# numz/ComfyUI-SeedVR2_VideoUpscaler

Hardware: NVIDIA H100
Metric: upscaled frames/sec SeedVR2-3B 720p->4K (higher is better)
Workload: dtype bf16

## Files before the change

comfyui-seedvr2_videoupscaler_b200/csrc/gemm.cu:

```cuda
#include <cuda.h>
#include <cuda_runtime.h>
#include <cuda_bf16.h>
#include <stdint.h>
#include <stdio.h>
#include <stdlib.h>

#include <type_traits>

#include "ptx.cuh"
#include "svr2_internal.h"

namespace svr2 {

constexpr int BLOCK_M = 128;
constexpr int BLOCK_K = 64;
constexpr int WGMMA_K = 16;

struct GemmParams {
  int M, N, K;
  int num_m_tiles, num_n_tiles, num_k_blocks;
  int band_h;
  int group_n;
  int a_mode;
  int tiles_w, tiles_h;
// ... 34 lines not shown
  const float* qk_weight;
  float qk_eps;
  int qkv_inner;
};

enum : int {
  EPI_BIAS = 1,
  EPI_GATE = 2,
  EPI_RESIDUAL = 4,
  EPI_SWIGLU = 8,
  EPI_GELU = 16,
  EPI_F32 = 32,
  EPI_SHUFFLE = 64,
  EPI_SILU = 128,
  EPI_ROWSTAT = 256,
  EPI_PEXP = 512,
  EPI_ROWSCALE = 1024,
};

template <int BLOCK_N, bool EPI_WG>
struct SmemLayout {
  static constexpr int kABytes = BLOCK_M * BLOCK_K * 2;
  static constexpr int kBBytes = BLOCK_N * BLOCK_K * 2;
  static constexpr int kStageBytes = kABytes + kBBytes;
  static constexpr int kTileCols = BLOCK_N < 32 ? 32 : BLOCK_N;
  static constexpr int kStagingBytes = EPI_WG ? BLOCK_M * kTileCols * 2 : 8 * 4096;
  static constexpr int kBudget = 232448 - kStagingBytes - 256 - 1024;
  static constexpr int kStages = kBudget / kStageBytes > 8 ? 8 : kBudget / kStageBytes;
  static constexpr int kStagingOffset = kStages * kStageBytes;
  static constexpr int kBarOffset = kStagingOffset + kStagingBytes;
  static constexpr int kTotal = kBarOffset + 256 + 1024;
};

__device__ __forceinline__ void acc_ld32(const float* acc, uint32_t idx, uint32_t (&v)[32]) {
  const float4* s = reinterpret_cast<const float4*>(acc + idx);
#pragma unroll
  for (int i = 0; i < 8; ++i) {
    const float4 t = s[i];
    v[4 * i] = __float_as_uint(t.x); v[4 * i + 1] = __float_as_uint(t.y);
    v[4 * i + 2] = __float_as_uint(t.z); v[4 * i + 3] = __float_as_uint(t.w);
  }
}

__device__ __forceinline__ void stat_acc(float4& a, const uint4& d) {
  const uint32_t w[4] = {d.x, d.y, d.z, d.w};
#pragma unroll
  for (int e = 0; e < 4; ++e) {
    const float lo = __uint_as_float(w[e] << 16), hi = __uint_as_float(w[e] & 0xffff0000u);
    if (e < 2) { a.x += lo + hi; a.y += lo * lo + hi * hi; }
    else { a.z += lo + hi; a.w += lo * lo + hi * hi; }
  }
}

__device__ __forceinline__ uint4 add_bf16x8(const uint4& a, const uint4& b) {
  const uint32_t aw[4] = {a.x, a.y, a.z, a.w}, bw[4] = {b.x, b.y, b.z, b.w};
  uint32_t o[4];
#pragma unroll
  for (int e = 0; e < 4; ++e)
    o[e] = pack_bf16x2(__uint_as_float(aw[e] << 16) + __uint_as_float(bw[e] << 16),
                       __uint_as_float(aw[e] & 0xffff0000u) + __uint_as_float(bw[e] & 0xffff0000u));
  return make_uint4(o[0], o[1], o[2], o[3]);
}

__device__ __forceinline__ void conv_tile(const GemmParams& p, int m_blk, int& t_o, int& th, int& tw) {
  const int full = p.T_out * p.band_h * p.tiles_w;
  const int band = m_blk / full;
// ... 50 lines not shown
    const int m = m_blk * BLOCK_M + row;
    d.valid = m < p.M;
    const int hw = p.shuf_H * p.shuf_W;
    const int f = m / hw, rr = m - f * hw, h = rr / p.shuf_W, w = rr - h * p.shuf_W;
    const int grp = (n_blk * BLOCK_N) / p.shuf_c;
    const int z = grp % p.shuf_z, y = (grp / p.shuf_z) & 1, x = grp / (p.shuf_z * 2);
    int t_out = f * p.shuf_z + z;
    if (p.shuf_drop) {
      if (f == 0 && z == 1) d.valid = 0;
      if (f > 0) t_out -= 1;
    }
    const int Wo = p.shuf_W * 2;
    const long long pix = (long long)(2 * h + x) * Wo + (2 * w + y);
    d.off = (long long)(t_out + p.out_t_pad) * p.out_frame_stride + pix * p.ldc + ((n_blk * BLOCK_N) % p.shuf_c);
    d.dup = (p.out_dup_head && t_out == 0 && d.valid) ? 1 : 0;
  } else if (p.a_mode == 0) {
    const int m = m_blk * BLOCK_M + row;
    d.valid = m < p.M;
    d.off = (long long)m * p.ldc + (long long)n_blk * n_cols;
  } else {
    int t_o, th, tw;
    conv_tile(p, m_blk, t_o, th, tw);
    const int rh = row / p.bw;
    const int h = th * p.bh + rh;
    const int w = tw * p.bw + (row - rh * p.bw);
    d.valid = (h < p.H_out) && (w < p.W_out);
    d.off = (long long)(t_o + p.out_t_pad) * p.out_frame_stride + ((long long)h * p.W_out + w) * p.ldc +
            (long long)n_blk * BLOCK_N;
    d.dup = (p.out_dup_head && t_o == 0 && d.valid) ? 1 : 0;
  }
  return d;
}

template <int BLOCK_N, int KIND, bool SWAP = false, int EPI_CT = -1>
__global__ void __launch_bounds__(kNumThreads, 1)
gemm_wgmma_kernel(const __grid_constant__ CUtensorMap tmap_a, const __grid_constant__ CUtensorMap tmap_b,
                  const __grid_constant__ CUtensorMap tmap_a2, const GemmParams p) {
  if (p.run_if != nullptr && *p.run_if == 0) return;
  constexpr bool EPI_WG = kEpiWG<KIND>;
  static_assert(EPI_WG || (!SWAP && EPI_CT < 0), "swap-AB and compile-time epilogues are KIND_BF16 only");
  using L = SmemLayout<BLOCK_N, EPI_WG>;
  constexpr int kStages = L::kStages;
  constexpr int ACC_STRIDE = BLOCK_N < 32 ? 32 : BLOCK_N;
  constexpr int ACC_LD = ACC_STRIDE + 4;
  static_assert(EPI_WG || BLOCK_M * ACC_LD * 4 <= L::kStagingOffset, "the accumulator tile overlays the operand ring");
  extern __shared__ uint8_t smem_raw[];
  uint8_t* smem = reinterpret_cast<uint8_t*>((reinterpret_cast<uintptr_t>(smem_raw) + 1023) & ~uintptr_t(1023));
  uint64_t* full_bar = reinterpret_cast<uint64_t*>(smem + L::kBarOffset);
  uint64_t* empty_bar = full_bar + kStages;
  uint64_t* acc_free = empty_bar + kStages;
  uint64_t* tile_full = acc_free + 1;
  uint64_t* tile_empty = acc_free + 2;
  const float* acc_s = reinterpret_cast<const float*>(smem);
  uint8_t* tile_s = smem + L::kStagingOffset;

  const int warp = threadIdx.x >> 5;
  const int lane = threadIdx.x & 31;

  if (warp == 0 && lane == 0) {
    tma_prefetch_desc(&tmap_a);
    tma_prefetch_desc(&tmap_b);
    if (p.extra_blocks) tma_prefetch_desc(&tmap_a2);
  }
  if (warp == 1 && lane == 0) {
    for (int i = 0; i < kStages; ++i) {
      mbar_init(&full_bar[i], 1);
      mbar_init(&empty_bar[i], 2);
    }
    if constexpr (EPI_WG) {
      mbar_init(tile_full, 256);
      mbar_init(tile_empty, 32 * kEpiWarps);
    } else {
      mbar_init(acc_free, 256);
    }
    fence_barrier_init();
  }
  __syncthreads();

  const int num_n_tiles = p.num_n_tiles;
  const int num_m_tiles = p.num_m_tiles;
  const int num_tiles = num_m_tiles * num_n_tiles;
  const int tile0 = (int)blockIdx.x;
  const int tile_step = (int)gridDim.x;

  if (warp == 0 || warp == 3) {
    if (lane == 0) {
      int stage = 0;
      uint32_t phase = 0;
      uint32_t g = (warp == 0) ? 0u : 1u;
      uint32_t it = 0;
      const int a_mode = p.a_mode;
      const int nkb = p.num_k_blocks;
      auto acquire = [&](uint8_t*& sa, uint64_t*& fb) -> bool {
        const bool mine = (g++ & 1u) == 0u;
        if (mine) {
          mbar_wait(&empty_bar[stage], phase ^ 1);
          sa = smem + stage * L::kStageBytes;
          fb = &full_bar[stage];
          mbar_expect_tx(fb, L::kStageBytes);
        }
        return mine;
      };
      auto advance = [&]() {
        if (++stage == kStages) { stage = 0; phase ^= 1; }
      };
      auto tile_start = [&]() {
        if (!EPI_WG && it > 0) mbar_wait(acc_free, (it - 1) & 1u);
        ++it;
      };
      if (a_mode == 0) {
        for (int tile = tile0; tile < num_tiles; tile += tile_step) {
          int m_blk, n_blk;
          tile_coords(tile, num_m_tiles, num_n_tiles, p.group_n, m_blk, n_blk);
          tile_start();
          const int m0 = m_blk * BLOCK_M, n0 = n_blk * BLOCK_N;
          for (int kb = 0; kb < nkb; ++kb) {
            uint8_t* sa; uint64_t* fb;
            if (acquire(sa, fb)) {
              tma_load_2d(sa, &tmap_a, fb, kb * BLOCK_K, m0);
// ... 59 lines not shown
  } else if (warp >= 4) {
    const int wg = (warp - 4) >> 2;
    int mstage = 0;
    uint32_t mphase = 0;
    uint32_t it = 0;
    auto mainloop = [&](int nkb, auto&& tail) {
      float d[BLOCK_N / 2];
#pragma unroll
      for (int i = 0; i < BLOCK_N / 2; ++i) d[i] = 0.f;
      const bool leader = (threadIdx.x & 127) == 0;
      int prev = -1;
      for (int kb = 0; kb < nkb; ++kb) {
        mbar_wait(&full_bar[mstage], mphase);
        const uint32_t a_addr = smem_u32(smem + mstage * L::kStageBytes);
        const uint64_t a_desc = wgmma_desc_kmajor_sw128(a_addr + wg * 64 * 128);
        const uint64_t b_desc = wgmma_desc_kmajor_sw128(a_addr + L::kABytes);
        wgmma_fence_regs(d);
        wgmma_fence();
#pragma unroll
        for (int k = 0; k < BLOCK_K / WGMMA_K; ++k)
          wgmma_ss<BLOCK_N>(d, a_desc + uint64_t(k * 2), b_desc + uint64_t(k * 2), (kb | k) != 0);
        wgmma_commit();
        wgmma_fence_regs(d);
        wgmma_wait<1>();
        if (prev >= 0 && leader) mbar_arrive(&empty_bar[prev]);
        prev = mstage;
        if (++mstage == kStages) { mstage = 0; mphase ^= 1; }
      }
      wgmma_wait<0>();
      wgmma_fence_regs(d);
      if (prev >= 0 && leader) mbar_arrive(&empty_bar[prev]);
      tail(d);
    };
    const int epi = EPI_CT >= 0 ? EPI_CT : p.epi;
    const __nv_bfloat16* __restrict__ bias = p.bias;
    if constexpr (EPI_WG) {
      const int r0 = wg * 64 + ((warp & 3) << 4);
      const uint32_t tbase = smem_u32(tile_s);
      const int lr = lane & 7, mj = lane >> 3;
      auto store_tile = [&](float (&d)[BLOCK_N / 2], int n_blk) {
        if (it > 0) mbar_wait(tile_empty, (it - 1) & 1u);
        if constexpr (SWAP) {
          const int co = n_blk * BLOCK_M + r0 + (lane >> 2);
          const bool has_bias = (epi & EPI_BIAS) != 0;
          const float b0 = (has_bias && co < p.N) ? __bfloat162float(bias[co]) : 0.f;
          const float b1 = (has_bias && co + 8 < p.N) ? __bfloat162float(bias[co + 8]) : 0.f;
          const int chunk = (r0 >> 3) + (mj & 1);
#pragma unroll
          for (int i = 0; i < BLOCK_N / 2; i += 8) {
            const int pix = (i >> 3) * 16 + ((mj >> 1) << 3) + lr;
            stmatrix_x4_trans(tbase + pix * 256 + ((chunk ^ swap_tile_swz(pix)) << 4),
                              pack_bf16x2(d[i] + b0, d[i + 1] + b0), pack_bf16x2(d[i + 2] + b1, d[i + 3] + b1),
                              pack_bf16x2(d[i + 4] + b0, d[i + 5] + b0), pack_bf16x2(d[i + 6] + b1, d[i + 7] + b1));
          }
        } else {
          constexpr int ROW_B = L::kTileCols * 2;
          constexpr int SWZ = (L::kTileCols / 8 < 8 ? L::kTileCols / 8 : 8) - 1;
          const int row = r0 + ((mj & 1) << 3) + lr;
          const int cn0 = n_blk * BLOCK_N + 2 * (lane & 3);
#pragma unroll
          for (int i = 0; i < BLOCK_N / 2; i += 8) {
            float x[8];
#pragma unroll
            for (int e = 0; e < 8; ++e) x[e] = d[i + e];
            if (epi & EPI_BIAS) {
              const int cn = cn0 + (i >> 3) * 16;
              const uint32_t bl = cn < p.N ? __ldg(reinterpret_cast<const unsigned int*>(bias + cn)) : 0u;
              const uint32_t bh = cn + 8 < p.N ? __ldg(reinterpret_cast<const unsigned int*>(bias + cn + 8)) : 0u;
              x[0] += __uint_as_float(bl << 16); x[1] += __uint_as_float(bl & 0xffff0000u);
              x[2] += __uint_as_float(bl << 16); x[3] += __uint_as_float(bl & 0xffff0000u);
              x[4] += __uint_as_float(bh << 16); x[5] += __uint_as_float(bh & 0xffff0000u);
              x[6] += __uint_as_float(bh << 16); x[7] += __uint_as_float(bh & 0xffff0000u);
            }
            const int chunk = (i >> 3) * 2 + (mj >> 1);
            stmatrix_x4(tbase + row * ROW_B + ((chunk ^ (row & SWZ)) << 4), pack_bf16x2(x[0], x[1]),
                        pack_bf16x2(x[2], x[3]), pack_bf16x2(x[4], x[5]), pack_bf16x2(x[6], x[7]));
          }
        }
        mbar_arrive(tile_full);
      };
      for (int tile = tile0; tile < num_tiles; tile += tile_step, ++it) {
        int m_blk, n_blk;
        tile_coords(tile, num_m_tiles, num_n_tiles, p.group_n, m_blk, n_blk);
        mainloop(conv_k_blocks(p, m_blk), [&](float (&d)[BLOCK_N / 2]) { store_tile(d, n_blk); });
      }
    } else {
      auto acc_to_smem = [&](float (&d)[BLOCK_N / 2]) {
        named_bar_sync(1, 256);
        float* acc_w = reinterpret_cast<float*>(smem);
        const int r0 = wg * 64 + ((warp & 3) << 4) + (lane >> 2);
#pragma unroll
        for (int i = 0; i < BLOCK_N / 2; i += 4) {
          const int col = (i >> 2) * 8 + 2 * (lane & 3);
          *reinterpret_cast<float2*>(acc_w + r0 * ACC_LD + col) = make_float2(d[i], d[i + 1]);
          *reinterpret_cast<float2*>(acc_w + (r0 + 8) * ACC_LD + col) = make_float2(d[i + 2], d[i + 3]);
        }
        named_bar_sync(1, 256);
      };
      constexpr bool IS_BF16 = KIND == KIND_BF16_RS;
      constexpr bool IS_PEXP = KIND == KIND_PEXP || KIND == KIND_PEXP_STAT;
      constexpr int N_COLS = KIND == KIND_SWIGLU ? ACC_STRIDE / 2 : ACC_STRIDE;
      constexpr int COLS_W = N_COLS >= 64 ? N_COLS / 2 : N_COLS;
      constexpr int PH_COLS = KIND == KIND_F32 ? 32 : (COLS_W < 64 ? COLS_W : 64);
      constexpr int CPR = KIND == KIND_F32 ? PH_COLS / 4 : PH_COLS / 8;
      constexpr int ROWS_PER_IT = 32 / CPR;
      constexpr int N_IT = 32 / ROWS_PER_IT;
      constexpr int kBatch = N_IT < 4 ? N_IT : 4;
      const int q = warp & 3;
      const int half = (warp - 4) >> 2;
      const int row = q * 32 + lane;
      const bool active = (N_COLS >= 64) || (half == 0);
      const int col_lo = (N_COLS >= 64) ? half * COLS_W : 0;
      uint8_t* slab = smem + L::kStagingOffset + (warp - 4) * 4096;
      const int n_lim = KIND == KIND_SWIGLU ? p.N / 2 : p.N;
      const float* __restrict__ gate = p.gate;
      const __nv_bfloat16* __restrict__ resid = p.residual;
      for (int tile = tile0; tile < num_tiles; tile += tile_step) {
// ... 511 lines not shown
  cuuint32_t bdim[5], estr[5];
  for (int i = 0; i < rank; ++i) {
    gdim[i] = dims[i];
    bdim[i] = box[i];
    estr[i] = 1;
    if (i > 0) gstr[i - 1] = strides_bytes[i - 1];
  }
  CUresult r = enc(map, CU_TENSOR_MAP_DATA_TYPE_BFLOAT16, rank, const_cast<void*>(base), gdim, gstr, bdim, estr,
                   CU_TENSOR_MAP_INTERLEAVE_NONE, CU_TENSOR_MAP_SWIZZLE_128B, CU_TENSOR_MAP_L2_PROMOTION_L2_256B,
                   CU_TENSOR_MAP_FLOAT_OOB_FILL_NONE);
  if (r != CUDA_SUCCESS) {
    char msg[256];
    snprintf(msg, sizeof msg, "cuTensorMapEncodeTiled failed (%d) rank=%d dims=%llu,%llu,%llu box=%u,%u,%u", (int)r,
             rank, (unsigned long long)dims[0], (unsigned long long)(rank > 1 ? dims[1] : 0),
             (unsigned long long)(rank > 2 ? dims[2] : 0), box[0], rank > 1 ? box[1] : 0, rank > 2 ? box[2] : 0);
    return set_error(SVR2_ERR_CUDA, msg);
  }
  return SVR2_OK;
}

constexpr int kMaxDevices = 64;
int current_device() {
  int dev = 0;
  cudaGetDevice(&dev);
  return (dev >= 0 && dev < kMaxDevices) ? dev : 0;
}
static int g_num_sms[kMaxDevices] = {};
int num_sms() {
  const int dev = current_device();
  if (!g_num_sms[dev]) cudaDeviceGetAttribute(&g_num_sms[dev], cudaDevAttrMultiProcessorCount, dev);
  return g_num_sms[dev];
}

template <int BLOCK_N, int KIND, bool SWAP = false, int EPI_CT = -1>
static int launch_gemm(const CUtensorMap& ta, const CUtensorMap& tb, const GemmParams& p_in, cudaStream_t stream,
                       const CUtensorMap* ta2_opt = nullptr) {
  const CUtensorMap& ta2 = ta2_opt ? *ta2_opt : ta;
  using L = SmemLayout<BLOCK_N, kEpiWG<KIND>>;
  auto kern = gemm_wgmma_kernel<BLOCK_N, KIND, SWAP, EPI_CT>;
  GemmParams p = p_in;
  {
    const long long b_tile_bytes = (long long)(SWAP ? BLOCK_M : BLOCK_N) * p.num_k_blocks * BLOCK_K * 2;
    long long g = (16LL << 20) / (b_tile_bytes > 0 ? b_tile_bytes : 1);
    if (g < 1) g = 1;
    if (g > p.num_n_tiles) g = p.num_n_tiles;
    p.group_n = (int)g;
  }
  static bool configured[kMaxDevices] = {};
  const int dev = current_device();
  if (!configured[dev]) {
    cudaError_t e = cudaFuncSetAttribute(kern, cudaFuncAttributeMaxDynamicSharedMemorySize, L::kTotal);
    if (e != cudaSuccess) return set_error(SVR2_ERR_CUDA, cudaGetErrorString(e));
    configured[dev] = true;
  }
  int tiles = p.num_m_tiles * p.num_n_tiles;
  int grid = tiles < num_sms() ? tiles : num_sms();
  if (grid <= 0) return SVR2_OK;
  kern<<<grid, kNumThreads, L::kTotal, stream>>>(ta, tb, ta2, p);
  cudaError_t e = cudaGetLastError();
  if (e != cudaSuccess) return set_error(SVR2_ERR_CUDA, cudaGetErrorString(e));
  return SVR2_OK;
}

static int dispatch_gemm(int block_n, const CUtensorMap& ta, const CUtensorMap& tb, const GemmParams& p,
                         cudaStream_t s, const CUtensorMap* ta2 = nullptr) {
  if (ta2) {
    switch (block_n) {
      case 256: return launch_gemm<256, KIND_BF16>(ta, tb, p, s, ta2);
      case 128: return launch_gemm<128, KIND_BF16>(ta, tb, p, s, ta2);
    }
    return set_error(SVR2_ERR_ARG, "fused shortcut: Cout must be >= 128");
  }
// ... 192 lines not shown
extern "C" int svr2_conv3d_stats_bf16(const void* x, int T_in_total, int H, int W, int Cin, const void* w, int Cout,
                                      int kt, int kh, int kw, int stride_t, int stride_hw, int pad_hw, int T_out,
                                      int epi_flags, const void* bias, const void* residual, void* y, int out_t_pad,
                                      int out_dup_head, int ldc, void* stat_partial, int64_t stat_bytes,
                                      int* stat_slots, void* stream) {
  if (!stat_slots) return set_error(SVR2_ERR_ARG, "svr2_conv3d_stats_bf16: stat_slots must not be NULL");
  return conv3d_impl(x, T_in_total, H, W, Cin, w, Cout, kt, kh, kw, stride_t, stride_hw, pad_hw, T_out, epi_flags, bias,
                     residual, y, out_t_pad, out_dup_head, ldc, stat_partial, stat_bytes, stat_slots, stream);
}

extern "C" int svr2_conv3d_shortcut_stats_bf16(const void* x, int T_in_total, int H, int W, int Cin, const void* w,
                                               int Cout, int kt, int kh, int kw, int T_out, const void* bias,
                                               const void* x2, int C2, void* y, int out_t_pad, int out_dup_head,
                                               void* stat_partial, int64_t stat_bytes, int* stat_slots, void* stream) {
  if (!x2 || C2 <= 0 || (C2 % 64)) return set_error(SVR2_ERR_ARG, "svr2_conv3d_shortcut_stats_bf16: x2 / C2 % 64");
  if (Cout < 128) return set_error(SVR2_ERR_ARG, "svr2_conv3d_shortcut_stats_bf16: Cout must be >= 128");
  return conv3d_impl(x, T_in_total, H, W, Cin, w, Cout, kt, kh, kw, 1, 1, 1, T_out, EPI_BIAS, bias, nullptr, y,
                     out_t_pad, out_dup_head, Cout, stat_partial, stat_bytes, stat_slots, stream, x2, C2);
}

static void conv_tile_shape(int Cout, int H_out, int W_out, bool* swap_out, int* bw_out, int* bh_out) {
  const bool swap = (Cout > 64 && Cout <= 128) && (long long)H_out * W_out >= 256;
  int bw = 16, bh = 8;
  if (swap) {
    bw = 32; bh = 8;
    if (W_out <= 16) { bw = 16; bh = 16; }
    if (W_out <= 8) { bw = 8; bh = 32; }
  } else {
    if (W_out >= 128 && H_out < 8) { bw = 128; bh = 1; }
    else if (W_out <= 8) { bw = 8; bh = 16; }
  }
  *swap_out = swap; *bw_out = bw; *bh_out = bh;
}
extern "C" int svr2_conv_stat_slots(int Cout, int H_out, int W_out) {
  bool swap;
  int bw, bh;
  conv_tile_shape(Cout, H_out, W_out, &swap, &bw, &bh);
  return ((W_out + bw - 1) / bw) * ((H_out + bh - 1) / bh) * (swap ? 2 : 4);
}

static int conv3d_impl(const void* x, int T_in_total, int H, int W, int Cin, const void* w, int Cout, int kt,
                       int kh, int kw, int stride_t, int stride_hw, int pad_hw, int T_out, int epi_flags,
                       const void* bias, const void* residual, void* y, int out_t_pad, int out_dup_head,
                       int ldc, void* stat_partial, int64_t stat_bytes, int* stat_slots_out, void* stream,
                       const void* x2, int C2) {
  if (Cin % 64) return set_error(SVR2_ERR_ARG, "svr2_conv3d_bf16: Cin must be a multiple of 64 (pad channels)");
  if (Cout % 8 || ldc % 8) return set_error(SVR2_ERR_ARG, "svr2_conv3d_bf16: Cout/ldc must be multiples of 8");
  if (stride_hw != 1 && stride_hw != 2) return set_error(SVR2_ERR_ARG, "stride_hw must be 1 or 2");
  const int H_out = stride_hw == 1 ? H : H / 2, W_out = stride_hw == 1 ? W : W / 2;
  if (stride_hw == 2 && ((H | W) & 1)) return set_error(SVR2_ERR_ARG, "stride-2 conv needs even H, W");
  bool swap;
  int bw, bh;
  conv_tile_shape(Cout, H_out, W_out, &swap, &bw, &bh);
  const int bn = swap ? 128 : pick_block_n(Cout, 0);
  CUtensorMap ta, tb;
  int rc;
  if (stride_hw == 1) {
    uint64_t d[4] = {(uint64_t)Cin, (uint64_t)W, (uint64_t)H, (uint64_t)T_in_total};
    uint64_t s[3] = {(uint64_t)Cin * 2, (uint64_t)W * Cin * 2, (uint64_t)H * W * Cin * 2};
    uint32_t b[4] = {BLOCK_K, (uint32_t)bw, (uint32_t)bh, 1};
    rc = make_tmap_bf16(&ta, x, 4, d, s, b);
  } else {
    uint64_t d[5] = {(uint64_t)Cin * 2, (uint64_t)W / 2, 2, (uint64_t)H / 2, (uint64_t)T_in_total};
    uint64_t s[4] = {(uint64_t)Cin * 4, (uint64_t)W * Cin * 2, (uint64_t)W * Cin * 4, (uint64_t)H * W * Cin * 2};
    uint32_t b[5] = {BLOCK_K, (uint32_t)bw, 1, (uint32_t)bh, 1};
    rc = make_tmap_bf16(&ta, x, 5, d, s, b);
  }
  if (rc) return rc;
  CUtensorMap ta2;
  if (x2) {
    uint64_t d[4] = {(uint64_t)C2, (uint64_t)W, (uint64_t)H, (uint64_t)T_out};
    uint64_t s2[3] = {(uint64_t)C2 * 2, (uint64_t)W * C2 * 2, (uint64_t)H * W * C2 * 2};
    uint32_t b[4] = {BLOCK_K, (uint32_t)bw, (uint32_t)bh, 1};
    rc = make_tmap_bf16(&ta2, x2, 4, d, s2, b);
    if (rc) return rc;
  }
  const int K = kt * kh * kw * Cin + (x2 ? C2 : 0);
  const bool fold = (epi_flags & SVR2_EPI_FOLD_HEAD) != 0;
  if (fold && (kt != 3 || x2 || Cout % bn))
    return set_error(SVR2_ERR_ARG, "svr2_conv3d_bf16: SVR2_EPI_FOLD_HEAD needs kt = 3, no shortcut and Cout a multiple of the n-tile");
  uint64_t db[2] = {(uint64_t)K, (uint64_t)(fold ? 2 * Cout : Cout)}, sb[1] = {(uint64_t)K * 2};
  uint32_t bb[2] = {BLOCK_K, (uint32_t)bn};
  rc = make_tmap_bf16(&tb, w, 2, db, sb, bb);
  if (rc) return rc;
  GemmParams p{};
  p.a_mode = stride_hw == 1 ? 1 : 2;
  p.bw = bw; p.bh = bh;
  p.tiles_w = (W_out + bw - 1) / bw;
  p.tiles_h = (H_out + bh - 1) / bh;
  p.taps_t = kt; p.taps_h = kh; p.taps_w = kw;
  p.cin_blocks = Cin / 64; p.cin = Cin;
  p.extra_blocks = x2 ? C2 / 64 : 0;
  p.pad_h = p.pad_w = pad_hw;
// ... 7 lines not shown
    if (bh == 1 && (bw == 256 || bw == 128) && kh == 3) {
      bhn = (8LL << 20) / (row_bytes > 0 ? row_bytes : 1);
      if (bhn < 2) bhn = 2;
      if (bhn > H_out) bhn = H_out;
    }
    p.band_h = (kt > 1) ? (int)bhn : (H_out + bh - 1) / bh;
  }
  p.M = T_out * p.tiles_w * p.tiles_h * BLOCK_M;
  p.N = Cout; p.K = K;
  p.num_m_tiles = T_out * p.tiles_w * p.tiles_h;
  p.num_n_tiles = (Cout + bn - 1) / bn;
  p.num_k_blocks = K / BLOCK_K;
  p.epi = epi_flags & (EPI_BIAS | EPI_RESIDUAL);
  p.ldc = ldc;
  p.out_frame_stride = (long long)H_out * W_out * ldc;
  p.out_t_pad = out_t_pad;
  p.out_dup_head = out_dup_head;
  if (fold) {
    p.fold_t = stride_t == 1 ? (T_out < 2 ? T_out : 2) : 1;
    p.fold_n = Cout;
  }
  p.bias = (const __nv_bfloat16*)bias;
  p.residual = (const __nv_bfloat16*)residual;
  p.out = y;
  if (stat_slots_out) {
    if (Cout % 8 || ldc != Cout) return set_error(SVR2_ERR_ARG, "conv stats: need Cout % 8 == 0 and ldc == Cout");
    const int slots = svr2_conv_stat_slots(Cout, H_out, W_out);
    *stat_slots_out = slots;
    if (!stat_partial) return SVR2_OK;
    const int64_t need = (int64_t)T_out * slots * (Cout / 8) * 16;
    if (stat_bytes < need) return set_error(SVR2_ERR_ARG, "conv stats: stat_partial buffer too small");
    p.stat_partial = (float4*)stat_partial;
    p.stat_slots = slots;
  }
  if (swap) return launch_gemm<256, KIND_BF16, true>(ta, tb, p, (cudaStream_t)stream, x2 ? &ta2 : nullptr);
  return dispatch_gemm(bn, ta, tb, p, (cudaStream_t)stream, x2 ? &ta2 : nullptr);
}

extern "C" int svr2_upsample_shuffle_bf16(const void* x, int F, int H, int W, int C, const void* w, const void* bias,
                                          int temporal, int drop_head, void* y, int out_t_pad, int out_dup_head,
                                          void* stream) {
  const int z = temporal ? 2 : 1;
  const int N = 4 * z * C, M = F * H * W;
  const int bn = C >= 256 ? 256 : 128;
  if (C % bn) return set_error(SVR2_ERR_ARG, "svr2_upsample_shuffle_bf16: C must be a multiple of 128");
  CUtensorMap ta, tb;
  uint64_t da[2] = {(uint64_t)C, (uint64_t)M}, sa[1] = {(uint64_t)C * 2};
  uint32_t ba[2] = {BLOCK_K, BLOCK_M};
  int rc = make_tmap_bf16(&ta, x, 2, da, sa, ba);
  if (rc) return rc;
  uint64_t db[2] = {(uint64_t)C, (uint64_t)N}, sb[1] = {(uint64_t)C * 2};
  uint32_t bb[2] = {BLOCK_K, (uint32_t)bn};
  rc = make_tmap_bf16(&tb, w, 2, db, sb, bb);
  if (rc) return rc;
  GemmParams p{};
  p.M = M; p.N = N; p.K = C;
  p.num_m_tiles = (M + BLOCK_M - 1) / BLOCK_M;
  p.num_n_tiles = N / bn;
  p.num_k_blocks = C / BLOCK_K;
  p.a_mode = 0;
  p.epi = EPI_SHUFFLE | (bias ? EPI_BIAS : 0);
  p.ldc = C;
  p.out_frame_stride = (long long)(2 * H) * (2 * W) * C;
  p.out_t_pad = out_t_pad;
  p.out_dup_head = out_dup_head;
  p.shuf_c = C; p.shuf_z = z; p.shuf_H = H; p.shuf_W = W;
// ... 6 lines not shown
```

comfyui-seedvr2_videoupscaler_b200/lib.py:

```python
from __future__ import annotations

import ctypes
import os
from ctypes import c_float, c_int, c_int64, c_void_p, POINTER

import torch

HERE = os.path.dirname(os.path.abspath(__file__))
LIB_PATH = os.environ.get("SVR2_LIB") or os.path.join(HERE, "csrc", "libsvr2.so")

EPI_BIAS, EPI_GATE, EPI_RESIDUAL, EPI_SWIGLU, EPI_GELU, EPI_F32, EPI_SILU = 1, 2, 4, 8, 16, 32, 128
EPI_ROWSTAT, EPI_PEXP, EPI_ROWSCALE, EPI_FOLD_HEAD = 256, 512, 1024, 2048

class ModelDesc(ctypes.Structure):
    _fields_ = [("variant", c_int), ("dim", c_int), ("heads", c_int), ("layers", c_int), ("mm_layers", c_int),
                ("txt_in_dim", c_int), ("in_ch", c_int), ("out_ch", c_int), ("mlp_kind", c_int), ("mlp_hidden", c_int),
                ("out_norm", c_int), ("last_vid_only", c_int), ("eps", c_float), ("timestep", c_float)]


class TensorDesc(ctypes.Structure):
    _fields_ = [("name", ctypes.c_char_p), ("data", c_void_p), ("dtype", c_int), ("rank", c_int), ("shape", c_int64 * 5)]


class DitGeometryDesc(ctypes.Structure):
    _fields_ = [(n, c_int) for n in ("n_win", "total", "max_len", "n_txt_rows", "nfreq", "rope_rows", "fuse_qkv")] + \
               [(n, c_void_p) for n in ("cu_seqlens", "row_src", "row_rope", "out_row_map", "tok_dst", "tok_rope",
                                        "txt_rows", "rope_cos", "rope_sin")]


_P = c_void_p
SIGNATURES = {
    "svr2_version": [],
    "svr2_device_check": [POINTER(c_int), POINTER(c_int), POINTER(c_int)],
    "svr2_create": [POINTER(c_void_p), c_int, POINTER(ModelDesc)],
    "svr2_destroy": [_P],
    "svr2_load_weights": [_P, POINTER(TensorDesc), ctypes.c_size_t, c_int],
    "svr2_workspace_bytes": [_P, c_int, c_int, c_int, c_int],
    "svr2_dit_forward": [_P, _P, _P, c_int, c_int, c_int, c_int, _P, _P],
    "svr2_dit_forward_ws": [_P, _P, _P, c_int, c_int, c_int, c_int, _P, _P, ctypes.c_size_t, _P],
    "svr2_dit_geometry": [_P, c_int, c_int, c_int, c_int, c_int, POINTER(DitGeometryDesc)],
    "svr2_vae_workspace_bytes": [_P, c_int, c_int, c_int, c_int, c_int],
    "svr2_vae_encode": [_P, _P, c_int, c_int, c_int, c_int, c_int, _P, _P, ctypes.c_size_t, _P],
    "svr2_vae_decode": [_P, _P, c_int, c_int, c_int, c_int, c_int, _P, _P, ctypes.c_size_t, _P],
    "svr2_vae_decode_frames_workspace_bytes": [_P, c_int, c_int, c_int, c_int, c_int],
    "svr2_vae_decode_frames": [_P, _P, c_int, c_int, c_int, c_int, c_int, c_int, _P, _P, ctypes.c_size_t, _P],
    "svr2_vae_tiled_workspace_bytes": [_P, c_int, c_int, c_int, c_int, c_int, c_int, c_int, c_int, c_int, c_int],
    "svr2_vae_encode_tiled": [_P, _P, c_int, c_int, c_int, c_int, c_int, c_int, c_int, c_int, c_int, _P, _P,
                              ctypes.c_size_t, _P],
    "svr2_vae_decode_tiled": [_P, _P, c_int, c_int, c_int, c_int, c_int, c_int, c_int, c_int, c_int, c_int, _P, _P,
                              ctypes.c_size_t, _P],
    "svr2_vae_last_launches": [_P],
    "svr2_linear_bf16": [_P, c_int64, _P, c_int64, c_int, c_int, c_int, c_int, _P, _P, _P, _P, c_int64, c_float, _P],
    "svr2_conv3d_bf16": [_P, c_int, c_int, c_int, c_int, _P, c_int, c_int, c_int, c_int, c_int, c_int, c_int, c_int,
                         c_int, _P, _P, _P, c_int, c_int, c_int, _P],
    "svr2_conv3d_stats_bf16": [_P, c_int, c_int, c_int, c_int, _P, c_int, c_int, c_int, c_int, c_int, c_int, c_int, c_int,
                               c_int, _P, _P, _P, c_int, c_int, c_int, _P, c_int64, POINTER(c_int), _P],
    "svr2_conv3d_shortcut_stats_bf16": [_P, c_int, c_int, c_int, c_int, _P, c_int, c_int, c_int, c_int, c_int, _P, _P, c_int,
                                        _P, c_int, c_int, _P, c_int64, POINTER(c_int), _P],
    "svr2_conv_stat_slots": [c_int, c_int, c_int],
    "svr2_groupnorm_from_stats_bf16": [_P, _P, c_int, c_int, c_int, _P, _P, c_float, c_int, c_int, c_int, _P, c_int, _P,
                                       _P],
    "svr2_upsample_shuffle_bf16": [_P, c_int, c_int, c_int, c_int, _P, _P, c_int, c_int, _P, c_int, c_int, _P],
    "svr2_attn_varlen_bf16": [_P, _P, _P, _P, _P, c_int, c_int, c_int, c_int, _P, _P],
    "svr2_rmsnorm_ada_bf16": [_P, _P, c_int, c_int, c_float, _P, _P, _P, c_int, _P],
    "svr2_qk_norm_rope_window_bf16": [_P, _P, _P, _P, _P, _P, c_int, _P, _P, _P, _P, c_float, c_int, c_int, _P, _P,
                                      _P, _P],
    "svr2_qk_norm_rope_rows_bf16": [_P, _P, _P, _P, _P, _P, c_int, _P, _P, _P, _P, c_float, _P, c_int, c_int, _P, _P,
                                    _P, _P],
    "svr2_linear_qkv_rope_bf16": [_P, c_int64, _P, c_int64, c_int, c_int, c_int, _P, _P, _P, _P, c_int, _P, c_float, _P,
                                  _P, _P, _P],
    "svr2_txt_window_mean_bf16": [_P, _P, c_int, c_int, c_int, _P],
    "svr2_patchify_bf16": [_P, _P, c_int, c_int, c_int, c_int, c_int, _P],
    "svr2_unpatchify_bf16": [_P, c_int, _P, c_int, c_int, c_int, c_int, _P],
    "svr2_groupnorm_bf16": [_P, _P, c_int, c_int, c_int, _P, _P, c_float, c_int, c_int, c_int, _P, c_int64, _P],
    "svr2_groupnorm_scratch_bytes": [c_int, c_int, c_int],
    "svr2_linear_ex_bf16": [_P, c_int64, _P, c_int64, c_int, c_int, c_int, c_int, _P, _P, _P, _P, c_int64, c_float, _P, _P,
                            c_int64, _P, _P],
    "svr2_rowstat_max": [_P, c_int, c_int64, _P, c_int, _P, _P],
    "svr2_pexp_stat_combine": [_P, c_int, c_int64, _P, _P, c_int, _P, _P],
    "svr2_rowstat_slots": [c_int],
    "svr2_rowstat_combine": [_P, c_int, c_int64, _P, c_int, _P],
    "svr2_transpose_bf16": [_P, c_int64, _P, c_int64, c_int, c_int, _P],
    "svr2_ncdhw_to_ndhwc_bf16": [_P, c_int, c_int, c_int, c_int, c_int, _P, c_int, c_int, c_float, _P],
    "svr2_ndhwc_to_ncdhw": [_P, c_int, c_int, c_int, c_int, c_int, _P, c_int, _P],
    "svr2_conv_tap_gather": [_P, c_int64, c_int, _P, c_int, c_int, c_int, _P, c_int, _P],
    "svr2_im2col3_bf16": [_P, c_int, c_int, c_int, c_int, c_int, _P, c_int, _P],
    "svr2_wavelet_level_bf16": [_P, _P, _P, _P, _P, c_int, c_int, c_int, c_int, c_int, _P],
    "svr2_wavelet_level_f32": [_P, c_int, _P, _P, _P, _P, c_int, c_int, c_int, c_int, c_int, _P],
    "svr2_hsv_scratch_bytes": [c_int64],
    "svr2_hsv_saturation_match_bf16": [_P, _P, _P, _P, c_int, c_int64, _P, c_int64, _P],
    "svr2_adain_bf16": [_P, _P, _P, c_int, c_int64, _P, _P],
    "svr2_rgb_to_lab_f32": [_P, _P, c_int, c_int64, _P],
# ... 14 lines not shown
    "svr2_resize_scratch_bytes": [c_int, c_int, c_int, c_int],
    "svr2_resize_bicubic_aa_bf16": [_P, c_int, c_int, c_int, c_int, c_int, c_int, _P, c_int, c_int, c_int, _P, c_int64,
                                    _P],
    "svr2_alpha_upscale_scratch_bytes": [c_int, c_int, c_int, c_int, c_int],
    "svr2_alpha_upscale": [_P, c_int, c_int, c_int, c_int, c_int, _P, c_int, c_int, _P, c_int, _P, c_int64, _P],
    "svr2_sobel_edges_f32": [_P, c_int, c_int, c_int, _P, _P, c_int64, _P],
    "svr2_sample_to_image_rgba_bf16": [_P, _P, c_int, c_int64, _P],
    "svr2_input_noise_bf16": [_P, _P, c_int, _P, c_int, c_int64, c_float, c_float, _P],
    "svr2_sr_condition_bf16": [_P, _P, _P, _P, _P, _P, c_int64, c_int, _P],
    "svr2_gguf_type_size": [c_int, POINTER(c_int), POINTER(c_int)],
    "svr2_gguf_dequant_f16": [c_int, _P, c_int64, _P, _P],
    "svr2_weight_expand_bf16": [c_int, _P, c_int64, c_int64, _P, c_int64, c_int64, c_int64, _P],
}

_lib = None


class Svr2Error(RuntimeError):
    pass


def load() -> ctypes.CDLL:
    global _lib
    if _lib is None:
        if not os.path.exists(LIB_PATH):
            raise Svr2Error(f"{LIB_PATH} not built — run `python __graft_entry__.py` (build()); "
                            "there is no CPU / PyTorch fallback")
        lib = ctypes.CDLL(LIB_PATH)
        lib.svr2_last_error.restype = ctypes.c_char_p
        lib.svr2_last_error.argtypes = []
        lib.svr2_engine_last_error.restype = ctypes.c_char_p
        lib.svr2_engine_last_error.argtypes = [c_void_p]
        for name, args in SIGNATURES.items():
            fn = getattr(lib, name)
            fn.restype = c_int64 if (name.endswith("_bytes") or name == "svr2_vae_last_launches") else (None if name == "svr2_destroy" else c_int)
            fn.argtypes = args
        _lib = lib
    return _lib


def _check(rc: int, what: str):
    if rc != 0:
        raise Svr2Error(f"{what} failed ({rc}): {load().svr2_last_error().decode()}")


def ptr(t):
    return None if t is None else c_void_p(t.data_ptr())


def stream():
    return c_void_p(torch.cuda.current_stream().cuda_stream)


KERNELS_PER_CALL = {"svr2_groupnorm_bf16": 3, "svr2_groupnorm_from_stats_bf16": 2,
                    "svr2_resize_bicubic_aa_bf16": 3,
                    "svr2_adain_bf16": 2,
                    "svr2_histogram_match_f32": 2,
                    "svr2_hsv_saturation_match_bf16": 3,
                    "svr2_alpha_upscale": 9,
                    "svr2_sobel_edges_f32": 5,
                    "svr2_input_noise_bf16": 1,
                    "svr2_sr_condition_bf16": 1}


class Profiler:

# ... 206 lines not shown
```

include/svr2.h:

```cpp
#ifndef SVR2_H_
#define SVR2_H_
#include <stddef.h>
#include <stdint.h>

#ifdef __cplusplus
extern "C" {
#endif

enum svr2_status {
  SVR2_OK = 0,
  SVR2_ERR_ARG = -1,
  SVR2_ERR_CUDA = -2,
  SVR2_ERR_ARCH = -3,
};

enum svr2_epilogue {
  SVR2_EPI_BIAS = 1,
  SVR2_EPI_GATE = 2,
  SVR2_EPI_RESIDUAL = 4,
  SVR2_EPI_SWIGLU = 8,
  SVR2_EPI_GELU = 16,
  SVR2_EPI_F32 = 32,
  SVR2_EPI_SILU = 128,
  SVR2_EPI_ROWSTAT = 256,
// ... 53 lines not shown
int svr2_vae_encode(svr2_t* engine, const void* x, int x_dtype, int T, int H, int W, int slice_frames, void* latent,
                    void* workspace, size_t workspace_bytes, void* stream);
int svr2_vae_decode(svr2_t* engine, const void* z, int z_dtype, int T, int h, int w, int slice_frames, void* sample,
                    void* workspace, size_t workspace_bytes, void* stream);
size_t svr2_vae_decode_frames_workspace_bytes(svr2_t* engine, int T, int h, int w, int slice_frames, int frames);
int svr2_vae_decode_frames(svr2_t* engine, const void* z, int z_dtype, int T, int h, int w, int slice_frames, int frames,
                           void* sample, void* workspace, size_t workspace_bytes, void* stream);
size_t svr2_vae_tiled_workspace_bytes(svr2_t* engine, int direction, int T, int H, int W, int tile_h, int tile_w,
                                      int overlap_h, int overlap_w, int slice_frames, int frames);
int svr2_vae_encode_tiled(svr2_t* engine, const void* x, int x_dtype, int T, int H, int W, int tile_h, int tile_w,
                          int overlap_h, int overlap_w, int slice_frames, void* latent, void* workspace,
                          size_t workspace_bytes, void* stream);
int svr2_vae_decode_tiled(svr2_t* engine, const void* z, int z_dtype, int T, int h, int w, int tile_h, int tile_w,
                          int overlap_h, int overlap_w, int slice_frames, int frames, void* sample, void* workspace,
                          size_t workspace_bytes, void* stream);
int64_t svr2_vae_last_launches(svr2_t* engine);

int svr2_linear_bf16(const void* a, int64_t lda, const void* w, int64_t ldw, int M, int N, int K, int epi_flags,
                     const void* bias, const float* gate, const void* residual, void* out, int64_t ldc,
                     float out_scale, void* stream);

int svr2_conv3d_bf16(const void* x, int T_in_total, int H, int W, int Cin, const void* w, int Cout, int kt, int kh,
                     int kw, int stride_t, int stride_hw, int pad_hw, int T_out, int epi_flags, const void* bias,
                     const void* residual, void* y, int out_t_pad, int out_dup_head, int ldc, void* stream);


int svr2_conv3d_stats_bf16(const void* x, int T_in_total, int H, int W, int Cin, const void* w, int Cout, int kt, int kh,
                           int kw, int stride_t, int stride_hw, int pad_hw, int T_out, int epi_flags, const void* bias,
                           const void* residual, void* y, int out_t_pad, int out_dup_head, int ldc, void* stat_partial,
                           int64_t stat_bytes, int* stat_slots, void* stream);

int svr2_conv_stat_slots(int Cout, int H_out, int W_out);

int svr2_conv3d_shortcut_stats_bf16(const void* x, int T_in_total, int H, int W, int Cin, const void* w, int Cout, int kt,
                                    int kh, int kw, int T_out, const void* bias, const void* x2, int C2, void* y,
                                    int out_t_pad, int out_dup_head, void* stat_partial, int64_t stat_bytes,
                                    int* stat_slots, void* stream);

int svr2_upsample_shuffle_bf16(const void* x, int F, int H, int W, int C, const void* w, const void* bias,
                               int temporal, int drop_head, void* y, int out_t_pad, int out_dup_head, void* stream);

int svr2_attn_varlen_bf16(const void* q, const void* k, const void* v, void* out, const int32_t* cu_seqlens,
                          int n_seq, int total, int heads, int max_seqlen, const int32_t* out_row_map,
                          void* stream);

int svr2_rmsnorm_ada_bf16(const void* x, void* y, int rows, int dim, float eps, const float* weight,
                          const float* scale, const float* shift, int mode, void* stream);

int svr2_qk_norm_rope_window_bf16(const void* qkv_vid, const void* qkv_txt, const int32_t* row_src,
                                  const int32_t* row_rope, const float* cos_tab, const float* sin_tab, int nfreq,
                                  const float* wq_vid, const float* wk_vid, const float* wq_txt, const float* wk_txt,
                                  float eps, int total, int heads, void* q, void* k, void* v, void* stream);
int svr2_qk_norm_rope_rows_bf16(const void* qkv_vid, const void* qkv_txt, const int32_t* row_src, const int32_t* row_rope,
                                const float* cos_tab, const float* sin_tab, int nfreq, const float* wq_vid,
                                const float* wk_vid, const float* wq_txt, const float* wk_txt, float eps,
                                const int32_t* row_list, int n_rows, int heads, void* q, void* k, void* v, void* stream);
int svr2_linear_qkv_rope_bf16(const void* a, int64_t lda, const void* w, int64_t ldw, int M, int heads, int K,
                              const int32_t* tok_dst, const int32_t* tok_rope, const float* cos_tab, const float* sin_tab,
                              int nfreq, const float* qk_weight, float eps, void* q, void* k, void* v, void* stream);


int svr2_txt_window_mean_bf16(const void* in, void* out, int n_win, int l, int dim, void* stream);

int svr2_patchify_bf16(const void* vid, void* out, int T, int H, int W, int C, int ld_out, void* stream);
int svr2_unpatchify_bf16(const void* in, int ld_in, void* out, int T, int H, int W, int C, void* stream);

// ... 94 lines not shown
```

Baseline: 1.515.

## Add slab mainloop reusing one input slab across three kh taps in conv GEMM

Adds a slab variant of the implicit-GEMM conv kernel for 3x3 stride-1 temporal convs with 256-wide tiles. Each TMA load fetches a (bh+2)-row input slab per (kt,kw,cin-block), and the three kh taps reuse it by offsetting the wgmma descriptor by one row. The activation and weight rings are split so the producer warps load independently. This cuts activation TMA traffic per tile roughly threefold, at the cost of fewer weight pipeline stages and a more complex ring scheme.

```diff
diff --git a/comfyui-seedvr2_videoupscaler_b200/csrc/gemm.cu b/comfyui-seedvr2_videoupscaler_b200/csrc/gemm.cu
--- a/comfyui-seedvr2_videoupscaler_b200/csrc/gemm.cu
+++ b/comfyui-seedvr2_videoupscaler_b200/csrc/gemm.cu
@@ -90,6 +90,21 @@
   static constexpr int kTotal = kBarOffset + 256 + 1024;
 };
 
+template <bool SWAP>
+struct SlabLayout : SmemLayout<256, true> {
+  using Base = SmemLayout<256, true>;
+  static constexpr int kWBytes = (SWAP ? BLOCK_M : 256) * BLOCK_K * 2;
+  static constexpr int kSBytes = (SWAP ? 32 * 10 : 16 * 10) * BLOCK_K * 2;
+  static constexpr int kSStages = SWAP ? 2 : 3;
+  static constexpr int kWStages = (Base::kBudget - kSStages * kSBytes) / kWBytes;
+  static constexpr int kStages = kWStages + kSStages;
+  static constexpr int kSlabOffset = kWStages * kWBytes;
+  static constexpr int kStagingOffset = kSlabOffset + kSStages * kSBytes;
+  static constexpr int kBarOffset = kStagingOffset + Base::kStagingBytes;
+  static constexpr int kTotal = kBarOffset + 256 + 1024;
+  static_assert(kWStages >= 3 && kSBytes % 1024 == 0 && kTotal <= 232448, "slab rings do not fit");
+};
+
 __device__ __forceinline__ void acc_ld32(const float* acc, uint32_t idx, uint32_t (&v)[32]) {
   const float4* s = reinterpret_cast<const float4*>(acc + idx);
 #pragma unroll
@@ -206,14 +221,16 @@
   return d;
 }
 
-template <int BLOCK_N, int KIND, bool SWAP = false, int EPI_CT = -1>
+template <int BLOCK_N, int KIND, bool SWAP = false, int EPI_CT = -1, bool SLAB = false>
 __global__ void __launch_bounds__(kNumThreads, 1)
 gemm_wgmma_kernel(const __grid_constant__ CUtensorMap tmap_a, const __grid_constant__ CUtensorMap tmap_b,
                   const __grid_constant__ CUtensorMap tmap_a2, const GemmParams p) {
   if (p.run_if != nullptr && *p.run_if == 0) return;
   constexpr bool EPI_WG = kEpiWG<KIND>;
   static_assert(EPI_WG || (!SWAP && EPI_CT < 0), "swap-AB and compile-time epilogues are KIND_BF16 only");
-  using L = SmemLayout<BLOCK_N, EPI_WG>;
+  static_assert(!SLAB || (KIND == KIND_BF16 && BLOCK_N == 256), "the slab mainloop is KIND_BF16 with 256-column tiles");
+  using S = SlabLayout<SWAP>;
+  using L = std::conditional_t<SLAB, S, SmemLayout<BLOCK_N, EPI_WG>>;
   constexpr int kStages = L::kStages;
   constexpr int ACC_STRIDE = BLOCK_N < 32 ? 32 : BLOCK_N;
   constexpr int ACC_LD = ACC_STRIDE + 4;
@@ -258,7 +275,67 @@
   const int tile_step = (int)gridDim.x;
 
   if (warp == 0 || warp == 3) {
-    if (lane == 0) {
+    if constexpr (SLAB) {
+      if (lane == 0) {
+        const bool wgt = warp == 0;
+        const int n_st = wgt ? S::kWStages : S::kSStages;
+        const int bar0 = wgt ? 0 : S::kWStages;
+        const int st_bytes = wgt ? S::kWBytes : S::kSBytes;
+        uint8_t* const ring = smem + (wgt ? 0 : S::kSlabOffset);
+        int stage = 0;
+        uint32_t phase = 0;
+        auto acquire = [&](uint32_t bytes, uint64_t*& fb) -> uint8_t* {
+          mbar_wait(&empty_bar[bar0 + stage], phase ^ 1);
+          fb = &full_bar[bar0 + stage];
+          mbar_expect_tx(fb, bytes);
+          uint8_t* s = ring + stage * st_bytes;
+          if (++stage == n_st) { stage = 0; phase ^= 1; }
+          return s;
+        };
+        const int bw = p.bw, bh = p.bh, taps_t = p.taps_t, cin_blocks = p.cin_blocks, cin = p.cin;
+        const uint32_t slab_bytes = bw * (bh + 2) * BLOCK_K * 2, box_bytes = bw * bh * BLOCK_K * 2;
+        for (int tile = tile0; tile < num_tiles; tile += tile_step) {
+          int m_blk, n_blk, t_o, th, tw;
+          tile_coords(tile, num_m_tiles, num_n_tiles, p.group_n, m_blk, n_blk);
+          conv_tile(p, m_blk, t_o, th, tw);
+          const int h0 = th * bh, w0 = tw * bw;
+          int n0 = n_blk * (SWAP ? BLOCK_M : BLOCK_N);
+          int taps = taps_t, kcol = 0;
+          if (t_o < p.fold_t) {
+            taps = t_o + 1;
+            kcol = t_o == 0 ? 2 * 9 * cin : 0;
+            n0 += p.fold_n;
+          }
+          uint64_t* fb;
+          for (int kt_ = 0; kt_ < taps; ++kt_) {
+            const int t_in = t_o * p.stride_t + taps_t - taps + kt_;
+            for (int kw_ = 0; kw_ < 3; ++kw_) {
+              for (int cb = 0; cb < cin_blocks; ++cb) {
+                if (wgt) {
+                  for (int kh_ = 0; kh_ < 3; ++kh_) {
+                    uint8_t* s = acquire(S::kWBytes, fb);
+                    tma_load_2d(s, &tmap_b, fb, kcol + ((kt_ * 3 + kh_) * 3 + kw_) * cin + cb * BLOCK_K, n0);
+                  }
+                } else {
+                  uint8_t* s = acquire(slab_bytes, fb);
+                  tma_load_4d(s, &tmap_a, fb, cb * BLOCK_K, w0 + kw_ - p.pad_w, h0 - p.pad_h, t_in);
+                }
+              }
+            }
+          }
+          kcol += taps * 9 * cin;
+          for (int cb = 0; cb < p.extra_blocks; ++cb) {
+            if (wgt) {
+              uint8_t* s = acquire(S::kWBytes, fb);
+              tma_load_2d(s, &tmap_b, fb, kcol + cb * BLOCK_K, n0);
+            } else {
+              uint8_t* s = acquire(box_bytes, fb);
+              tma_load_4d(s, &tmap_a2, fb, cb * BLOCK_K, w0, h0, t_o);
+            }
+          }
+        }
+      }
+    } else if (lane == 0) {
       int stage = 0;
       uint32_t phase = 0;
       uint32_t g = (warp == 0) ? 0u : 1u;
@@ -384,6 +461,55 @@
       if (prev >= 0 && leader) mbar_arrive(&empty_bar[prev]);
       tail(d);
     };
+    int wstage = 0, sstage = 0;
+    uint32_t wphase = 0, sphase = 0;
+    auto mainloop_slab = [&](int nkb, auto&& tail) {
+      float d[BLOCK_N / 2];
+#pragma unroll
+      for (int i = 0; i < BLOCK_N / 2; ++i) d[i] = 0.f;
+      const bool leader = (threadIdx.x & 127) == 0;
+      const int nkb_taps = nkb - p.extra_blocks;
+      const uint32_t row_bytes = p.bw * BLOCK_K * 2;
+      const uint32_t w_ring = smem_u32(smem), s_ring = smem_u32(smem + S::kSlabOffset);
+      int prev_w = -1, prev_s = -1, kh = 0;
+      for (int kb = 0; kb < nkb; ++kb) {
+        mbar_wait(&full_bar[wstage], wphase);
+        if (kh == 0) mbar_wait(&full_bar[S::kWStages + sstage], sphase);
+        const uint32_t w_addr = w_ring + wstage * S::kWBytes;
+        const uint32_t s_addr = s_ring + sstage * S::kSBytes + kh * row_bytes;
+        const uint64_t a_desc = wgmma_desc_kmajor_sw128((SWAP ? w_addr : s_addr) + wg * 64 * 128);
+        const uint64_t b_desc = wgmma_desc_kmajor_sw128(SWAP ? s_addr : w_addr);
+        wgmma_fence_regs(d);
+        wgmma_fence();
+#pragma unroll
+        for (int k = 0; k < BLOCK_K / WGMMA_K; ++k)
+          wgmma_ss<BLOCK_N>(d, a_desc + uint64_t(k * 2), b_desc + uint64_t(k * 2), (kb | k) != 0);
+        wgmma_commit();
+        wgmma_fence_regs(d);
+        wgmma_wait<1>();
+        if (leader) {
+          if (prev_w >= 0) mbar_arrive(&empty_bar[prev_w]);
+          if (prev_s >= 0) mbar_arrive(&empty_bar[S::kWStages + prev_s]);
+        }
+        prev_w = wstage;
+        if (++wstage == S::kWStages) { wstage = 0; wphase ^= 1; }
+        prev_s = -1;
+        if (kh == 2 || kb >= nkb_taps) {
+          prev_s = sstage;
+          if (++sstage == S::kSStages) { sstage = 0; sphase ^= 1; }
+          kh = 0;
+        } else {
+          ++kh;
+        }
+      }
+      wgmma_wait<0>();
+      wgmma_fence_regs(d);
+      if (leader) {
+        if (prev_w >= 0) mbar_arrive(&empty_bar[prev_w]);
+        if (prev_s >= 0) mbar_arrive(&empty_bar[S::kWStages + prev_s]);
+      }
+      tail(d);
+    };
     const int epi = EPI_CT >= 0 ? EPI_CT : p.epi;
     const __nv_bfloat16* __restrict__ bias = p.bias;
     if constexpr (EPI_WG) {
@@ -434,7 +560,9 @@
       for (int tile = tile0; tile < num_tiles; tile += tile_step, ++it) {
         int m_blk, n_blk;
         tile_coords(tile, num_m_tiles, num_n_tiles, p.group_n, m_blk, n_blk);
-        mainloop(conv_k_blocks(p, m_blk), [&](float (&d)[BLOCK_N / 2]) { store_tile(d, n_blk); });
+        auto store = [&](float (&d)[BLOCK_N / 2]) { store_tile(d, n_blk); };
+        if constexpr (SLAB) mainloop_slab(conv_k_blocks(p, m_blk), store);
+        else mainloop(conv_k_blocks(p, m_blk), store);
       }
     } else {
       auto acc_to_smem = [&](float (&d)[BLOCK_N / 2]) {
@@ -1012,12 +1140,12 @@
   return g_num_sms[dev];
 }
 
-template <int BLOCK_N, int KIND, bool SWAP = false, int EPI_CT = -1>
+template <int BLOCK_N, int KIND, bool SWAP = false, int EPI_CT = -1, bool SLAB = false>
 static int launch_gemm(const CUtensorMap& ta, const CUtensorMap& tb, const GemmParams& p_in, cudaStream_t stream,
                        const CUtensorMap* ta2_opt = nullptr) {
   const CUtensorMap& ta2 = ta2_opt ? *ta2_opt : ta;
-  using L = SmemLayout<BLOCK_N, kEpiWG<KIND>>;
-  auto kern = gemm_wgmma_kernel<BLOCK_N, KIND, SWAP, EPI_CT>;
+  using L = std::conditional_t<SLAB, SlabLayout<SWAP>, SmemLayout<BLOCK_N, kEpiWG<KIND>>>;
+  auto kern = gemm_wgmma_kernel<BLOCK_N, KIND, SWAP, EPI_CT, SLAB>;
   GemmParams p = p_in;
   {
     const long long b_tile_bytes = (long long)(SWAP ? BLOCK_M : BLOCK_N) * p.num_k_blocks * BLOCK_K * 2;
@@ -1276,6 +1404,17 @@
   }
   *swap_out = swap; *bw_out = bw; *bh_out = bh;
 }
+static bool conv_slab(int Cout, int kt, int kh, int kw, int stride_hw, int H_out, int W_out) {
+  bool swap;
+  int bw, bh;
+  conv_tile_shape(Cout, H_out, W_out, &swap, &bw, &bh);
+  return stride_hw == 1 && kt > 1 && kh == 3 && kw == 3 && bh > 1 && (swap || pick_block_n(Cout, 0) == 256);
+}
+extern "C" int svr2_conv_mainloop(int Cin, int Cout, int kt, int kh, int kw, int stride_hw, int H, int W) {
+  if (Cin <= 0 || Cin % 64 || Cout <= 0 || (stride_hw != 1 && stride_hw != 2))
+    return set_error(SVR2_ERR_ARG, "svr2_conv_mainloop: Cin must be a positive multiple of 64, stride_hw 1 or 2");
+  return conv_slab(Cout, kt, kh, kw, stride_hw, stride_hw == 1 ? H : H / 2, stride_hw == 1 ? W : W / 2) ? 1 : 0;
+}
 extern "C" int svr2_conv_stat_slots(int Cout, int H_out, int W_out) {
   bool swap;
   int bw, bh;
@@ -1297,12 +1436,13 @@
   int bw, bh;
   conv_tile_shape(Cout, H_out, W_out, &swap, &bw, &bh);
   const int bn = swap ? 128 : pick_block_n(Cout, 0);
+  const bool slab = conv_slab(Cout, kt, kh, kw, stride_hw, H_out, W_out);
   CUtensorMap ta, tb;
   int rc;
   if (stride_hw == 1) {
     uint64_t d[4] = {(uint64_t)Cin, (uint64_t)W, (uint64_t)H, (uint64_t)T_in_total};
     uint64_t s[3] = {(uint64_t)Cin * 2, (uint64_t)W * Cin * 2, (uint64_t)H * W * Cin * 2};
-    uint32_t b[4] = {BLOCK_K, (uint32_t)bw, (uint32_t)bh, 1};
+    uint32_t b[4] = {BLOCK_K, (uint32_t)bw, (uint32_t)(slab ? bh + 2 : bh), 1};
     rc = make_tmap_bf16(&ta, x, 4, d, s, b);
   } else {
     uint64_t d[5] = {(uint64_t)Cin * 2, (uint64_t)W / 2, 2, (uint64_t)H / 2, (uint64_t)T_in_total};
@@ -1376,6 +1516,13 @@
     if (stat_bytes < need) return set_error(SVR2_ERR_ARG, "conv stats: stat_partial buffer too small");
     p.stat_partial = (float4*)stat_partial;
     p.stat_slots = slots;
+  }
+  const CUtensorMap* ta2p = x2 ? &ta2 : nullptr;
+  if (slab) {
+    if (swap) return launch_gemm<256, KIND_BF16, true, -1, true>(ta, tb, p, (cudaStream_t)stream, ta2p);
+    if (p.epi == EPI_BIAS && !x2)
+      return launch_gemm<256, KIND_BF16, false, EPI_BIAS, true>(ta, tb, p, (cudaStream_t)stream);
+    return launch_gemm<256, KIND_BF16, false, -1, true>(ta, tb, p, (cudaStream_t)stream, ta2p);
   }
   if (swap) return launch_gemm<256, KIND_BF16, true>(ta, tb, p, (cudaStream_t)stream, x2 ? &ta2 : nullptr);
   return dispatch_gemm(bn, ta, tb, p, (cudaStream_t)stream, x2 ? &ta2 : nullptr);
diff --git a/comfyui-seedvr2_videoupscaler_b200/lib.py b/comfyui-seedvr2_videoupscaler_b200/lib.py
--- a/comfyui-seedvr2_videoupscaler_b200/lib.py
+++ b/comfyui-seedvr2_videoupscaler_b200/lib.py
@@ -7,7 +7,8 @@
 import torch
 
 HERE = os.path.dirname(os.path.abspath(__file__))
-LIB_PATH = os.environ.get("SVR2_LIB") or os.path.join(HERE, "csrc", "libsvr2.so")
+DEFAULT_LIB_PATH = os.path.join(HERE, "csrc", "libsvr2.so")
+LIB_PATH = os.environ.get("SVR2_LIB") or DEFAULT_LIB_PATH
 
 EPI_BIAS, EPI_GATE, EPI_RESIDUAL, EPI_SWIGLU, EPI_GELU, EPI_F32, EPI_SILU = 1, 2, 4, 8, 16, 32, 128
 EPI_ROWSTAT, EPI_PEXP, EPI_ROWSCALE, EPI_FOLD_HEAD = 256, 512, 1024, 2048
@@ -58,6 +59,7 @@
     "svr2_conv3d_shortcut_stats_bf16": [_P, c_int, c_int, c_int, c_int, _P, c_int, c_int, c_int, c_int, c_int, _P, _P, c_int,
                                         _P, c_int, c_int, _P, c_int64, POINTER(c_int), _P],
     "svr2_conv_stat_slots": [c_int, c_int, c_int],
+    "svr2_conv_mainloop": [c_int, c_int, c_int, c_int, c_int, c_int, c_int, c_int],
     "svr2_groupnorm_from_stats_bf16": [_P, _P, c_int, c_int, c_int, _P, _P, c_float, c_int, c_int, c_int, _P, c_int, _P,
                                        _P],
     "svr2_upsample_shuffle_bf16": [_P, c_int, c_int, c_int, c_int, _P, _P, c_int, c_int, _P, c_int, c_int, _P],
@@ -138,6 +140,9 @@
         lib.svr2_engine_last_error.restype = ctypes.c_char_p
         lib.svr2_engine_last_error.argtypes = [c_void_p]
         for name, args in SIGNATURES.items():
+            fn = getattr(lib, name, None)
+            if fn is None and LIB_PATH != DEFAULT_LIB_PATH:
+                continue
             fn = getattr(lib, name)
             fn.restype = c_int64 if (name.endswith("_bytes") or name == "svr2_vae_last_launches") else (None if name == "svr2_destroy" else c_int)
             fn.argtypes = args
diff --git a/include/svr2.h b/include/svr2.h
--- a/include/svr2.h
+++ b/include/svr2.h
@@ -109,6 +109,8 @@
 
 int svr2_conv_stat_slots(int Cout, int H_out, int W_out);
 
+int svr2_conv_mainloop(int Cin, int Cout, int kt, int kh, int kw, int stride_hw, int H, int W);
+
 int svr2_conv3d_shortcut_stats_bf16(const void* x, int T_in_total, int H, int W, int Cin, const void* w, int Cout, int kt,
                                     int kh, int kw, int T_out, const void* bias, const void* x2, int C2, void* y,
                                     int out_t_pad, int out_dup_head, void* stat_partial, int64_t stat_bytes,
```

Result: faster. 1.564, median of 6 (+3.3%).
